# shz9/viprs

Hardware: AMD Instinct MI355X
Metric: SNP-updates/sec/E-step (1M SNPs, ~1700 LD blocks) (higher is better)
Workload: dtype f32

## Files before the change

include/viprs_hip.h:

```cpp
#ifndef VIPRS_HIP_H
#define VIPRS_HIP_H

#include <stdint.h>

#ifdef __cplusplus
extern "C" {
#endif

enum viprs_float_dtype { VIPRS_F32 = 0, VIPRS_F64 = 1 };
enum viprs_ld_dtype {
    VIPRS_LD_I8 = 0, VIPRS_LD_I16 = 1, VIPRS_LD_I32 = 2, VIPRS_LD_I64 = 3,
    VIPRS_LD_F32 = 4, VIPRS_LD_F64 = 5
};
enum viprs_indptr_dtype { VIPRS_IP_I32 = 0, VIPRS_IP_I64 = 1 };

enum viprs_status {
    VIPRS_OK = 0,
    VIPRS_EINVAL = -1,
    VIPRS_ELAYOUT = -2,
    VIPRS_EDEVICE = -3,
    VIPRS_ENOMEM = -4,
    VIPRS_EUNSUPPORTED = -5
};

// ... 104 lines not shown
int viprs_state_reset_column(viprs_state* state, int g, double pi);

int viprs_state_set_groups(viprs_state* state, int n_groups, const int64_t* group_start);
int viprs_state_prep_groups(viprs_state* state, int n, const double* params);
int viprs_state_sums_groups_begin(viprs_state* state, int n, const double* rows);
int viprs_state_sums_groups_end(viprs_state* state, double* out);
int viprs_state_prep_mixture_groups(viprs_state* state, int n, const double* params);
int viprs_state_sums_mixture_groups_begin(viprs_state* state, int n, const double* rows);
int viprs_state_sums_mixture_groups_end(viprs_state* state, double* out);
int viprs_state_prep_grid_groups(viprs_state* state, int n, const double* params);
int viprs_state_sums_grid_groups_begin(viprs_state* state, int n, const double* rows);
int viprs_state_sums_grid_groups_end(viprs_state* state, double* out);
int viprs_state_set_group_columns(viprs_state* state, int n_groups, int width, const uint8_t* active);

int viprs_state_commit_groups(viprs_state* dst, const viprs_state* src, int n, const int32_t* pairs);

#define VIPRS_COMM_ID_BYTES 128
typedef struct viprs_comm viprs_comm;
int viprs_comm_unique_id(void* id);
int viprs_comm_create(viprs_comm** comm, const void* id, int rank, int world_size, int device);
int viprs_comm_destroy(viprs_comm* comm);
int viprs_comm_rank(const viprs_comm* comm, int* rank, int* world_size);
int viprs_comm_allreduce(viprs_comm* comm, double* vec, int n, int group);
int viprs_comm_allgather(viprs_comm* comm, const double* send, int64_t n, double* recv);
int viprs_comm_barrier(viprs_comm* comm);
int viprs_state_set_comm(viprs_state* state, viprs_comm* comm);
int viprs_device_synchronize(int device);

int viprs_plan_last_kernel_ms(viprs_plan* plan, int which, double* ms);
int viprs_plan_timing_reset(viprs_plan* plan);
int viprs_plan_timing_history(viprs_plan* plan, int which, double* ms, int capacity, int* n);
int viprs_plan_last_math_modes(const viprs_plan* plan, int* mask);
int viprs_plan_last_skipped(viprs_plan* plan, int64_t* n_skipped);

int viprs_plan_dot(viprs_plan* plan, int float_dtype, int n_cols, const void* b_host, void* y_host,
                   double dq_scale, int include_diagonal);
int viprs_state_dot(viprs_state* state, int field, double dq_scale, int include_diagonal, void* y_host);
int viprs_plan_last_dot_ms(viprs_plan* plan, double* ms);

int viprs_plan_create_synthetic(viprs_plan** plan, int64_t n_blocks, const int64_t* sizes, const float* pw,
                                const float* uf0, const float* uf1, const float* sa, const float* sf, int ld_dtype,
                                int low_memory, int device);
int viprs_synthetic_ld_host(int64_t n_blocks, const int64_t* sizes, const float* pw, const float* uf0, const float* uf1,
                            const float* sa, const float* sf, int ld_dtype, int low_memory, void* out, int64_t capacity);

#ifdef __cplusplus
}
#endif
#endif
```

viprs_amd/_lib.py:

```python
import ctypes
import os

_HERE = os.path.dirname(os.path.abspath(__file__))
LIB_PATH = os.environ.get("VIPRS_HIP_LIB") or os.path.join(_HERE, "lib", "libviprs_hip.so")

F32, F64 = 0, 1
LD_I8, LD_I16, LD_I32, LD_I64, LD_F32, LD_F64 = range(6)
IP_I32, IP_I64 = 0, 1
MATH_EXACT, MATH_FAST = 0, 1
BLOCK_DENSE_SYM, BLOCK_DENSE_UPPER, BLOCK_RAGGED = 0, 1, 2
MODEL_SPIKE_SLAB, MODEL_MIXTURE, MODEL_GRID = 0, 1, 2
(FIELD_STD_BETA, FIELD_U_LOGS, FIELD_SQRT_HALF_VAR_TAU, FIELD_MU_MULT, FIELD_LOG_NULL_PI,
 FIELD_VAR_GAMMA, FIELD_VAR_MU, FIELD_ETA, FIELD_Q, FIELD_ETA_DIFF) = range(10)
(INFO_M, INFO_NNZ, INFO_N_BLOCKS, INFO_N_DENSE, INFO_N_RAGGED, INFO_MAX_BLOCK, INFO_LD_BYTES_DEVICE,
 INFO_LD_ELEM_SIZE, INFO_DEVICE, INFO_LOW_MEMORY, INFO_N_CU, INFO_UPPER_MIRRORED) = range(12)

OK, EINVAL, ELAYOUT, EDEVICE, ENOMEM, EUNSUPPORTED = 0, -1, -2, -3, -4, -5
N_SUMS = 11
COMM_ID_BYTES = 128


class ViprsHipError(RuntimeError):
    """A libviprs_hip call failed (device error, unsupported configuration...)."""

# ... 54 lines not shown
    "viprs_state_set_log_var_tau": (_i, [_vp, _vp]),
    "viprs_state_prep_mixture": (_i, [_vp, _vp, _vp, _vp, _d, _d, _d]),
    "viprs_state_sums_mixture_begin": (_i, [_vp, _d]),
    "viprs_state_sums_mixture_end": (_i, [_vp, _vp]),
    "viprs_state_prep_columns": (_i, [_vp, _i, _vp]),
    "viprs_state_sums_columns_begin": (_i, [_vp, _i, _vp]),
    "viprs_state_sums_columns_end": (_i, [_vp, _vp]),
    "viprs_state_reset_column": (_i, [_vp, _i, _d]),
    "viprs_state_set_groups": (_i, [_vp, _i, _vp]),
    "viprs_state_prep_groups": (_i, [_vp, _i, _vp]),
    "viprs_state_sums_groups_begin": (_i, [_vp, _i, _vp]),
    "viprs_state_sums_groups_end": (_i, [_vp, _vp]),
    "viprs_state_prep_mixture_groups": (_i, [_vp, _i, _vp]),
    "viprs_state_sums_mixture_groups_begin": (_i, [_vp, _i, _vp]),
    "viprs_state_sums_mixture_groups_end": (_i, [_vp, _vp]),
    "viprs_state_prep_grid_groups": (_i, [_vp, _i, _vp]),
    "viprs_state_sums_grid_groups_begin": (_i, [_vp, _i, _vp]),
    "viprs_state_sums_grid_groups_end": (_i, [_vp, _vp]),
    "viprs_state_set_group_columns": (_i, [_vp, _i, _i, _vp]),
    "viprs_state_commit_groups": (_i, [_vp, _vp, _i, _vp]),
    "viprs_comm_unique_id": (_i, [_vp]),
    "viprs_comm_create": (_i, [ctypes.POINTER(_vp), _vp, _i, _i, _i]),
    "viprs_comm_destroy": (_i, [_vp]),
    "viprs_comm_rank": (_i, [_vp, ctypes.POINTER(_i), ctypes.POINTER(_i)]),
    "viprs_comm_allreduce": (_i, [_vp, _vp, _i, _i]),
    "viprs_comm_allgather": (_i, [_vp, _vp, _i64, _vp]),
    "viprs_comm_barrier": (_i, [_vp]),
    "viprs_state_set_comm": (_i, [_vp, _vp]),
    "viprs_device_synchronize": (_i, [_i]),
    "viprs_plan_create_synthetic": (_i, [ctypes.POINTER(_vp), _i64, _vp, _vp, _vp, _vp, _vp, _vp, _i, _i, _i]),
    "viprs_synthetic_ld_host": (_i, [_i64, _vp, _vp, _vp, _vp, _vp, _vp, _i, _i, _vp, _i64]),
    "viprs_plan_last_kernel_ms": (_i, [_vp, _i, ctypes.POINTER(_d)]),
    "viprs_plan_last_skipped": (_i, [_vp, _pi64]),
    "viprs_plan_last_math_modes": (_i, [_vp, ctypes.POINTER(_i)]),
    "viprs_plan_timing_reset": (_i, [_vp]),
    "viprs_plan_timing_history": (_i, [_vp, _i, ctypes.POINTER(_d), _i, ctypes.POINTER(_i)]),
    "viprs_plan_dot": (_i, [_vp, _i, _i, _vp, _vp, _d, _i]),
    "viprs_state_dot": (_i, [_vp, _i, _d, _i, _vp]),
    "viprs_plan_last_dot_ms": (_i, [_vp, ctypes.POINTER(_d)]),
}

EXPORTED_SYMBOLS = tuple(_PROTOS)

for _name, (_res, _args) in _PROTOS.items():
    _fn = getattr(lib, _name)
    _fn.restype = _res
    _fn.argtypes = _args


def last_error():
    msg = lib.viprs_last_error()
    return msg.decode("utf-8", "replace") if msg else ""


def check(rc):
    if rc == OK:
        return
    msg = last_error()
    if rc == ELAYOUT:
        raise ViprsLayoutError(msg)
    if rc == EINVAL:
        raise ValueError(msg)
    if rc == ENOMEM:
        raise MemoryError(msg)
    if rc == EUNSUPPORTED:
        raise NotImplementedError(msg)
    raise ViprsHipError(msg)


def build_flags():
    return (lib.viprs_build_flags() or b"").decode()


def device_count():
    n = _i(0)
    rc = lib.viprs_device_count(ctypes.byref(n))
    return n.value if rc == OK else 0
```

viprs_amd/csrc/abi_estep.hip:

```cpp
#include "internal.h"

using namespace viprs;

namespace {

__global__ void sweep_prologue_kernel(int32_t* counters, int n_counters, unsigned long long* skipped,
                                      unsigned long long* granules, int64_t n_granules) {
    const int64_t i = (int64_t)blockIdx.x * blockDim.x + threadIdx.x;
    if (i < n_counters) counters[i] = 0;
    if (i == 0) { skipped[0] = 0ull; skipped[1] = 0ull; }
    for (int64_t k = i; k < n_granules; k += (int64_t)gridDim.x * blockDim.x) granules[k] = 0ull;
}

hipError_t clear_stale_skip_count(viprs_plan* P) {
    if (!P->skip_count_in_place) return hipSuccess;
    P->skip_count_in_place = false;
    return hipMemsetAsync(P->d_skipped.p, 0, sizeof(unsigned long long), P->stream);
}

template <typename T>
EStepArgs<T> make_args(viprs_state* S, double dq) {
    viprs_plan* P = S->plan;
    EStepArgs<T> A{};
    A.skipped = P->d_skipped.p;
// ... 62 lines not shown

bool use_band(const viprs_plan* P) {
    const char* f = getenv("VIPRS_BAND");
    if ((f && !atoi(f)) || P->ragged_h.empty()) return false;
    if (P->ld_dtype != VIPRS_LD_F32 && P->ld_dtype != VIPRS_LD_I8 && P->ld_dtype != VIPRS_LD_I16) return false;
    return band_ring_panels(P) <= kBandMaxRingPanels;
}

int launch_band_u(viprs_plan* P, const EStepArgs<float>& A, int model) {
    switch (P->ld_dtype) {
        case VIPRS_LD_F32: return launch_band<float>(P, A, model);
        case VIPRS_LD_I8: return launch_band<int8_t>(P, A, model);
        case VIPRS_LD_I16: return launch_band<int16_t>(P, A, model);
        default: return fail(VIPRS_EINVAL, "band schedule with unsupported LD dtype");
    }
}

int run_spike_slab(viprs_state* S, double dq) {
    viprs_plan* P = S->plan;
    HIP_TRY(hipSetDevice(P->device));
    const bool dense_only = S->float_dtype == VIPRS_F32 && !P->dense_h.empty() && P->ragged_h.empty();
    if (!dense_only) {
        const int64_t ng = P->n_granule_rows * kPanel;
        const unsigned grid = (unsigned)std::max<int64_t>(1, std::min<int64_t>((ng + 255) / 256, 1024));
        sweep_prologue_kernel<<<grid, 256, 0, P->stream>>>(P->d_counters.p, kPlanCounters, P->d_skipped.p, P->d_granules.p, ng);
        HIP_TRY(hipGetLastError());
        P->skip_count_in_place = true;
    } else {
        HIP_TRY(clear_stale_skip_count(P));
    }
    P->math_used = 0;
    hipEvent_t* ev = P->ev.data() + 4 * (P->sweeps % viprs_plan::kRing);
    P->ev_dense_only[P->sweeps % viprs_plan::kRing] = dense_only;
    if (!dense_only) HIP_TRY(hipEventRecord(ev[0], P->stream));
    int rc = VIPRS_OK;
    if (S->float_dtype == VIPRS_F32) {
        EStepArgs<float> A = make_args<float>(S, dq);
        if (!P->dense_h.empty()) {
            P->pending_start_event = ev[2];
            switch (P->ld_dtype) {
                case VIPRS_LD_F32: rc = launch_panel<float>(P, A, kPanelSpikeSlab); break;
                case VIPRS_LD_I8: rc = launch_panel<int8_t>(P, A, kPanelSpikeSlab); break;
                case VIPRS_LD_I16: rc = launch_panel<int16_t>(P, A, kPanelSpikeSlab); break;
                default: rc = fail(VIPRS_EINVAL, "dense schedule with unsupported LD dtype"); break;
            }
            if (rc != VIPRS_OK) { P->pending_start_event = nullptr; return rc; }
            HIP_TRY(hipEventRecord(ev[3], P->stream));
            P->host_t1[P->sweeps % viprs_plan::kRing] = host_clock_ms();
        }
        if (use_band(P)) rc = launch_band_u(P, A, kBandSpikeSlab);
        else if (!P->ragged_h.empty()) rc = launch_generic_u<float>(P, A, kGenSpikeSlab, false);
    } else {
        EStepArgs<double> A = make_args<double>(S, dq);
        if (!P->dense_h.empty()) { P->host_t0[P->sweeps % viprs_plan::kRing] = host_clock_ms(); HIP_TRY(hipEventRecord(ev[2], P->stream)); }
        rc = launch_tile_f64_u(P, A, kGenSpikeSlab, true);
        if (rc == VIPRS_OK && !P->dense_h.empty()) { HIP_TRY(hipEventRecord(ev[3], P->stream)); P->host_t1[P->sweeps % viprs_plan::kRing] = host_clock_ms(); }
        if (rc == VIPRS_OK) rc = launch_tile_f64_u(P, A, kGenSpikeSlab, false);
    }
    if (rc != VIPRS_OK) return rc;
    if (!dense_only) HIP_TRY(hipEventRecord(ev[1], P->stream));
    P->sweeps++;
    return VIPRS_OK;
}

static int sweep_prologue(viprs_plan* P, int n_models = 1) {
    P->skip_count_in_place = true;
// ... 5 lines not shown
    const unsigned grid = (unsigned)std::max<int64_t>(1, std::min<int64_t>((ng + 255) / 256, 1024));
    sweep_prologue_kernel<<<grid, 256, 0, P->stream>>>(P->d_counters.p, kPlanCounters, P->d_skipped.p, P->d_granules.p, ng);
    HIP_TRY(hipGetLastError());
    return VIPRS_OK;
}

static bool use_grid_mfma(const viprs_plan* P, int width) {
    if ((int64_t)P->m * std::max(1, width) >= (1LL << 31)) return false;
    if (P->grid_mfma >= 0) return P->grid_mfma != 0;
    return (int64_t)P->dense_h.size() * 8 >= (int64_t)P->n_cu * 3;
}

static int launch_grid_mfma_u(viprs_plan* P, const EStepArgs<float>& A) {
    switch (P->ld_dtype) {
        case VIPRS_LD_F32: return launch_grid_mfma<float>(P, A);
        case VIPRS_LD_I8: return launch_grid_mfma<int8_t>(P, A);
        case VIPRS_LD_I16: return launch_grid_mfma<int16_t>(P, A);
        default: return fail(VIPRS_EINVAL, "dense schedule with unsupported LD dtype");
    }
}

int run_generic_model(viprs_state* S, double dq, int model, const int32_t* d_active, int n_active,
                      const int32_t* h_active) {
    viprs_plan* P = S->plan;
    HIP_TRY(hipSetDevice(P->device));
    const bool panel_only = S->float_dtype == VIPRS_F32 && !P->dense_h.empty() && P->ragged_h.empty() &&
                            ((model == kGenMixture && S->width <= kPanelWideMaxK) || (model == kGenGrid && !use_grid_mfma(P, S->width)));
    int rc = panel_only ? VIPRS_OK : sweep_prologue(P, model == kGenGrid ? n_active : 1);
    if (rc != VIPRS_OK) return rc;
    if (panel_only) HIP_TRY(clear_stale_skip_count(P));
    P->math_used = 0;
    hipEvent_t* ev = P->ev.data() + 4 * (P->sweeps % viprs_plan::kRing);
    P->ev_dense_only[P->sweeps % viprs_plan::kRing] = true;
    {
        const bool panel_ok0 = S->float_dtype == VIPRS_F32 && !P->dense_h.empty() && (model == kGenGrid || S->width <= kPanelWideMaxK);
        if (panel_ok0) P->pending_start_event = ev[2];
        else { P->host_t0[P->sweeps % viprs_plan::kRing] = host_clock_ms(); HIP_TRY(hipEventRecord(ev[2], P->stream)); }
    }
    if (S->float_dtype == VIPRS_F32) {
        EStepArgs<float> A = make_args<float>(S, dq);
        A.active = d_active;
        A.n_active = n_active;
        if (model == kGenGrid && !S->group_cols_h.empty()) {
            A.blk_group = S->d_blk_group.p;
            A.group_cols = S->d_group_cols.p;
        }
        const int64_t lists_per_chunk = (int64_t)S->n_groups * kGroupListStride;
        const bool panel_ok = !P->dense_h.empty() && (model == kGenGrid || S->width <= kPanelWideMaxK);
        if (panel_ok && model == kGenMixture) {
            rc = launch_panel_u(P, A, S->width <= kPanelMaxK ? kPanelMixture : kPanelMixtureWide);
        } else if (panel_ok && model == kGenGrid && use_grid_mfma(P, A.width)) {
            for (int off = 0; off < n_active && rc == VIPRS_OK; off += kGridModels) {
                EStepArgs<float> Ac = A;
                Ac.active = d_active + off;
                Ac.n_active = std::min(kGridModels, n_active - off);
                if (A.group_cols) Ac.group_lists = S->d_group_lists.p + (off / kGridModels) * lists_per_chunk;
                if (off > 0) rc = sweep_prologue(P, 1);
                if (rc == VIPRS_OK) rc = launch_grid_mfma_u(P, Ac);
            }
        } else if (panel_ok && model == kGenGrid) {
            A.granules = P->d_granules.p;
            rc = launch_panel_u(P, A, kPanelGridColumn);
        } else {
            rc = launch_generic_u<float>(P, A, model, true);
        }
        if (rc == VIPRS_OK) {
// ... 270 lines not shown
```

viprs_amd/csrc/abi_plan.hip:

```cpp
#include "internal.h"
#include <chrono>

using namespace viprs;

namespace {
thread_local std::string g_err;
viprs::BuildFlagsRegistrar tu_build_flags_(VIPRS_TU_BUILD_FLAGS);
}

namespace viprs {
int fail(int code, const std::string& msg) {
    g_err = msg;
    return code;
}
SchedConfig& sched_config() {
    static SchedConfig c;
    return c;
}
static std::string& build_flags_registry() {
    static std::string s;
    return s;
}
void register_build_flags(const char* flags) {
    std::string& all = build_flags_registry();
// ... 362 lines not shown
    auto last = g_gate_plan.find(P->device);
    if (it != g_gate_event.end() && (last == g_gate_plan.end() || last->second != P))
        HIP_TRY(hipStreamWaitEvent(P->stream, it->second, 0));
    return VIPRS_OK;
}
void team_launch_forget(const viprs_plan* P) {
    std::lock_guard<std::mutex> lock(g_gate_mutex);
    auto last = g_gate_plan.find(P->device);
    if (last != g_gate_plan.end() && last->second == P) g_gate_plan.erase(last);
}
int team_launch_done(viprs_plan* P) {
    std::lock_guard<std::mutex> lock(g_gate_mutex);
    auto it = g_gate_event.find(P->device);
    if (it == g_gate_event.end()) {
        hipEvent_t e = nullptr;
        HIP_TRY(hipEventCreateWithFlags(&e, hipEventDisableTiming));
        it = g_gate_event.emplace(P->device, e).first;
    }
    HIP_TRY(hipEventRecord(it->second, P->stream));
    g_gate_plan[P->device] = P;
    return VIPRS_OK;
}
int plan_create_generated(viprs_plan** out, int64_t m, const int32_t* lb, const std::vector<int64_t>& ip64, int ld_dtype,
                          int low_memory, int device, const std::function<int(void*)>& fill) {
    return plan_create_impl(out, m, lb, ip64, nullptr, ld_dtype, low_memory, device, nullptr, &fill);
}
}

extern "C" {

const char* viprs_last_error(void) { return g_err.c_str(); }
const char* viprs_version(void) { return "viprs_amd 0.1.0 (gfx950)"; }
const char* viprs_build_flags(void) { return build_flags_registry().c_str(); }

int viprs_device_count(int* count) {
    if (!count) return fail(VIPRS_EINVAL, "count is null");
    int n = 0;
    hipError_t e = hipGetDeviceCount(&n);
    if (e != hipSuccess) { *count = 0; return fail(VIPRS_EDEVICE, hipGetErrorString(e)); }
    *count = n;
    return VIPRS_OK;
}

int viprs_host_fingerprint(const void* data, int64_t n_bytes, uint64_t* out) {
    if (!out || n_bytes < 0 || (n_bytes > 0 && !data)) return fail(VIPRS_EINVAL, "bad argument");
    const unsigned char* b = static_cast<const unsigned char*>(data);
    uint64_t h = 0x9e3779b97f4a7c15ull ^ (uint64_t)n_bytes;
    auto mix = [&](const unsigned char* p, int64_t n) {
        int64_t i = 0;
        for (; i + 8 <= n; i += 8) {
            uint64_t w;
            std::memcpy(&w, p + i, 8);
            h = (h ^ w) * 0xff51afd7ed558ccdull;
            h ^= h >> 32;
        }
        for (; i < n; ++i) { h = (h ^ p[i]) * 0x100000001b3ull; }
    };
    constexpr int64_t kEdge = 4096, kSamples = 256, kWin = 64;
    if (n_bytes <= 2 * kEdge + kSamples * kWin) {
        mix(b, n_bytes);
    } else {
        mix(b, kEdge);
        mix(b + n_bytes - kEdge, kEdge);
        const int64_t step = (n_bytes - kWin) / kSamples;
        for (int64_t k = 0; k < kSamples; ++k) mix(b + k * step, kWin);
    }
// ... 181 lines not shown
```

viprs_amd/csrc/estep_panel.h:

```cpp
#pragma once
#include <type_traits>

#include "device_math.h"
#include "kernels_common.h"

#ifndef PANEL_MIN_WAVES
#define PANEL_MIN_WAVES 2
#endif

namespace viprs {

#ifdef VIPRS_SWEEP_TRACE
__device__ unsigned long long g_sweep_trace[1 << 15][4];
__device__ unsigned int g_sweep_trace_n;
#endif

#ifdef VIPRS_PANEL_PROFILE
#define PPROF(slot, cond) do { if (TEAM && item == 0 && member < 2 && lane == 0 && p < 64 && (cond)) s_pprof[p][slot] = (unsigned)wall_clock64(); } while (0)
#else
#define PPROF(slot, cond) do { } while (0)
#endif

template <typename U> __device__ __forceinline__ float4 load4(const U* p);
template <> __device__ __forceinline__ float4 load4<float>(const float* p) {
// ... 131 lines not shown
template <typename U, int CPL, bool FULL, int DEPTH = kStripRowsInFlight, bool MIXED = false>
__device__ __forceinline__ void strip_update(const U* __restrict__ rowp, int stride, int last_row, float avec,
                                             float* __restrict__ lq_c, float fvec = 1.0f) {
    static_assert(kPanel % DEPTH == 0, "panel must be a whole number of prefetch groups");
    float qv[CPL];
#pragma unroll
    for (int i = 0; i < CPL; ++i) qv[i] = lq_c[i];
    RawRow<U, CPL> buf[DEPTH];
#pragma unroll
    for (int k = 0; k < DEPTH; ++k)
        buf[k] = load_raw<U, CPL>(rowp + (int64_t)(FULL ? k : min(k, last_row)) * stride);
#pragma unroll 1
    for (int g = 0; g < kPanel / DEPTH - 1; ++g) {
#pragma unroll
        for (int k = 0; k < DEPTH; ++k) {
            const RawRow<U, CPL> v = buf[k];
            const int rn = DEPTH * (g + 1) + k;
            buf[k] = load_raw<U, CPL>(rowp + (int64_t)(FULL ? rn : min(rn, last_row)) * stride);
            const float a = MIXED ? fvec * rl(avec, DEPTH * g + k) : rl(avec, DEPTH * g + k);
#pragma unroll
            for (int i = 0; i < CPL; ++i) qv[i] = __builtin_fmaf(v.get(i), a, qv[i]);
            __builtin_amdgcn_sched_barrier(0);
        }
    }
#pragma unroll
    for (int k = 0; k < DEPTH; ++k) {
        const RawRow<U, CPL> v = buf[k];
        const float a = MIXED ? fvec * rl(avec, kPanel - DEPTH + k) : rl(avec, kPanel - DEPTH + k);
#pragma unroll
        for (int i = 0; i < CPL; ++i) qv[i] = __builtin_fmaf(v.get(i), a, qv[i]);
    }
#pragma unroll
    for (int i = 0; i < CPL; ++i) lq_c[i] = qv[i];
}

__device__ __forceinline__ float diag_lower_update(const float* __restrict__ tile, float edvec, float sv, int lane) {
#pragma unroll 16
    for (int jr = 0; jr < kPanel; ++jr) {
        const float t = __builtin_fmaf(tile[jr * kPanel + lane], rl(edvec, jr), sv);
        sv = lane < jr ? t : sv;
    }
    return sv;
}

template <bool EXACT>
struct SpikeSlabModel {
    static constexpr bool kLaneParallel = false;
    struct In { float mm, beta, sv, ulog, eta_old; };
    static __device__ __forceinline__ In load(const EStepArgs<float>& A, int64_t j, bool live) {
        In in;
        in.mm = live ? A.mu_mult[j] : 0.0f;
        in.beta = live ? A.std_beta[j] : 0.0f;
        in.sv = live ? A.shvt[j] : 0.0f;
        in.ulog = live ? A.u_logs[j] : 0.0f;
        in.eta_old = live ? A.eta[j] : 0.0f;
        return in;
    }
    static constexpr bool kHasSkip = true;
    template <int LOOKUP>
    static __device__ __forceinline__ float delta(const In& in, float q, const ExpTab& tab, int sel) {
        float mu, gamma, d;
        snp_update<EXACT, LOOKUP>(in.mm, in.beta, in.sv, in.ulog, in.eta_old, q, tab, mu, gamma, d, sel);
        return d;
    }
    template <int LOOKUP>
    static __device__ __forceinline__ bool update(const In& in, float q, const ExpTab& tab, float& d, int sel) {
// ... 45 lines not shown
        gamma = EXACT ? sigmoid_exact<LOOKUP>(u, tab, sel) : sigmoid_fast(u);
        d = gamma * mu - in.eta_old;
    }
    static constexpr bool kHasSkip = false;
    template <int LOOKUP>
    static __device__ __forceinline__ float delta(const In& in, float q, const ExpTab& tab, int sel) {
        float mu, gamma, d;
        core<LOOKUP>(in, q, tab, mu, gamma, d, sel);
        return d;
    }
    template <int LOOKUP>
    static __device__ __forceinline__ bool update(const In& in, float q, const ExpTab& tab, float& d, int sel) {
        d = delta<LOOKUP>(in, q, tab, sel);
        return true;
    }
    template <bool TEAM>
    static __device__ __forceinline__ float finish(const EStepArgs<float>& A, int64_t j, const In& in, float q,
                                                   const ExpTab& tab, bool live, bool writer, bool& skipped,
                                                   float* d_out = nullptr) {
        float mu, gamma, d;
        core<kLookupPerLane>(in, q, tab, mu, gamma, d, 0);
        if (d_out) *d_out = live ? d : 0.0f;
        if (live && writer) {
            A.var_mu[j] = mu;
            A.var_gamma[j] = gamma;
            A.eta_diff[j] = d;
            if (TEAM) stage_store(A.eta_out + j, in.eta_old + d); else A.eta[j] = in.eta_old + d;
        }
        skipped = false;
        return live ? A.dq * d : 0.0f;
    }
};

template <typename MODEL> struct IsGridColumn : std::false_type {};
template <bool EXACT> struct IsGridColumn<GridColumnModel<EXACT>> : std::true_type {};

template <bool EXACT, int LOOKUP>
__device__ __forceinline__ float softmax_exp(float x, const ExpTab& tab, int sel = 0) {
    if constexpr (EXACT) return expf_glibc_nonpos<LOOKUP>(x, tab, sel);
    else return expf_fast_nonpos(x);
}
template <bool EXACT>
__device__ __forceinline__ float softmax_div(float e, float ssum) {
    if constexpr (EXACT) return e / ssum;
    else return e * __builtin_amdgcn_rcpf(ssum);
}

template <bool EXACT = true>
struct MixtureModel {
    static constexpr bool kExact = EXACT;
    static constexpr bool kLaneParallel = true;
    struct In { float mm[kPanelMaxK], sv[kPanelMaxK], ulog[kPanelMaxK]; float lnp, beta, eta_old; int K; };
    static __device__ __forceinline__ In load(const EStepArgs<float>& A, int64_t j, bool live) {
        In in;
        in.K = A.width;
#pragma unroll
        for (int k = 0; k < kPanelMaxK; ++k) {
            const bool on = live && k < in.K;
            const int64_t idx = on ? j * in.K + k : 0;
            in.mm[k] = on ? A.mu_mult[idx] : 0.0f;
            in.sv[k] = on ? A.shvt[idx] : 0.0f;
            in.ulog[k] = on ? A.u_logs[idx] : 0.0f;
        }
        in.lnp = live ? A.log_null_pi[j] : 0.0f;
        in.beta = live ? A.std_beta[j] : 0.0f;
        in.eta_old = live ? A.eta[j] : 0.0f;
// ... 66 lines not shown
    static __device__ __forceinline__ In load(const EStepArgs<float>& A, int64_t j, bool live) {
        In in;
        in.K = A.width;
        in.lnp = live ? A.log_null_pi[j] : 0.0f;
        in.beta = live ? A.std_beta[j] : 0.0f;
        in.eta_old = live ? A.eta[j] : 0.0f;
        return in;
    }
};
template <typename M, typename = void> struct is_wide_mixture { static constexpr bool value = false; };
template <typename M> struct is_wide_mixture<M, std::enable_if_t<M::kWide>> { static constexpr bool value = true; };

constexpr int kFormSym = 1, kFormMirror = 2;

template <typename U, typename MODEL, int FORM, int NW, bool TEAM, int CPL>
__device__ __forceinline__ void panel_role(const EStepArgs<float>& A0, const int qcap, float* __restrict__ smem, const int wg) {
    constexpr bool MIR = FORM == kFormMirror;
    constexpr bool SUMS = FORM != kFormSym;
    constexpr bool kDiagInLds = !MODEL::kLaneParallel;
    constexpr bool kMixLds = MODEL::kLaneParallel;
    constexpr bool kStageDiag = kDiagInLds || kMixLds;
    float* lq = smem;
    float* la = smem + qcap;
    float* lT = la + 2 * kPanel;
    float* lTo = lT + 2 * kPanel * kPanel;
    float* lmx = lTo + kPanel * kPanel;
    float* led = lmx + ((MODEL::kLaneParallel && !is_wide_mixture<MODEL>::value) ? kMixLdsFloats : 0);
    float* ls = led + 2 * kPanel;
#ifdef PANEL_TEAM_STRIP_DEPTH
    constexpr int kDepth = TEAM ? PANEL_TEAM_STRIP_DEPTH : kStripRowsInFlight;
#else
    constexpr int kDepth = TEAM ? (kPanel / RawRow<U, CPL>::kWords < kPanel ? kPanel / RawRow<U, CPL>::kWords : kPanel) : kStripRowsInFlight;
#endif
    __shared__ int s_blk;
    __shared__ int s_tdone;
    __shared__ int s_ddone;

    const int tid = threadIdx.x;
    const int wave = __builtin_amdgcn_readfirstlane(tid >> 6);
    const int lane = tid & 63;
    const U* __restrict__ ldd = static_cast<const U*>(A0.ld_dense);
    ExpTab tab;
    tab.init();
    unsigned long long my_skipped = 0;
    const float dq = A0.dq;
    const int n_models = max(1, A0.n_active);

    constexpr int kSW = kPanel * CPL;
    const int TS = TEAM ? A0.team_size : 1;
    const int team = TEAM ? wg / TS : 0;
    const int member = TEAM ? wg % TS : 0;
    int team_iter = 0;

    for (;;) {
        int item;
        if (TEAM) {
            item = team + team_iter * A0.n_teams;
            ++team_iter;
        } else {
            if (tid == 0) {
                int it = atomicAdd(A0.counter, 1);
                if (A0.bottom_mod > 0 && it < A0.n_blocks * n_models) {
                    const bool bottom = (wg % A0.bottom_mod) == A0.bottom_mod - 1;
                    it = bottom ? A0.n_blocks * n_models - 1 - atomicAdd(A0.counter + 2, 1) : atomicAdd(A0.counter + 1, 1);
                }
                s_blk = it;
// ... 430 lines not shown
                        v[g] = load4<U>(base + (int64_t)min(row_base + row, b - 1) * stride + (p + 1) * kPanel + tcol);
                    }
                    float4 w[kGroups];
                    {
#pragma unroll
                        for (int g = 0; g < kGroups; ++g) {
                            const int row = 4 * min(uw + g * (NW - 1), kPanel / 4 - 1) + trow;
                            w[g] = load4<U>(base + (int64_t)min(p * kPanel + row, b - 1) * stride + (p + 1) * kPanel + tcol);
                        }
                    }
                    if (MIR && p > 0) {
                        while (*reinterpret_cast<volatile int*>(&s_ddone) < p) __builtin_amdgcn_s_sleep(1);
                    }
#pragma unroll
                    for (int g = 0; g < kGroups; ++g) {
                        const int i = uw + g * (NW - 1);
                        if (i < kPanel / 4) *reinterpret_cast<float4*>(T + (4 * i + trow) * kPanel + tcol) = v[g];
                    }
                    {
                        while (*reinterpret_cast<volatile int*>(&s_tdone) < p + 1) __builtin_amdgcn_s_sleep(1);
#pragma unroll
                        for (int g = 0; g < kGroups; ++g) {
                            const int i = uw + g * (NW - 1);
                            if (i < kPanel / 4) *reinterpret_cast<float4*>(lTo + (4 * i + trow) * kPanel + tcol) = w[g];
                        }
                    }
                }
                };
                const int pp = p - 1;
                const int rr0 = pp * kPanel;
                const int last_row = min(kPanel, b - rr0) - 1;
                const float avec = p > 0 ? la[(pp & 1) * kPanel + lane] : 0.0f;
                const int nstrips = (bpad + kSW - 1) / kSW;
                const bool any_a = __ballot(avec != 0.0f) != 0;
                const float edvec = (MIR && p > 0) ? led[(pp & 1) * kPanel + lane] : 0.0f;
                const bool any_ed = MIR && __ballot(edvec != 0.0f) != 0;
                const int s_pri = ((p + 1) * kPanel) / kSW;
                const int n_mine = (nstrips - member + TS - 1) / TS;
                auto do_strip = [&](int k) {
                    int st = member + k * TS, kl = k;
                    if (TEAM) {
                        const int k_pri = (s_pri % TS == member) ? (s_pri - member) / TS : 0;
                        kl = (k + k_pri) % n_mine;
                        st = member + kl * TS;
                    }
                    const int c = st * kSW + CPL * lane;
                    float* __restrict__ lq_c = lq + (TEAM ? kl * kSW + CPL * lane : c);
                    const int cp = c >> 6;
#if defined(PANEL_TIMING_NO_SECOND_PASS) && PANEL_TIMING_NO_SECOND_PASS + 0 >= 2
                    const bool active = (c < b) && cp > p;
#else
                    const bool active = (c < b) && cp != pp && cp != p;
#endif
                    auto hand_off = [&]() {
                        if (TEAM && st == s_pri && p + 1 < np && p + 1 >= 2) {
                            __builtin_amdgcn_wave_barrier();
                            const float v = lq[loc((p + 1) * kPanel + lane)];
                            const unsigned long long g =
                                ((unsigned long long)(A.tag_base + (unsigned)(p + 2)) << 32) | (unsigned long long)__float_as_uint(v);
                            __hip_atomic_store(gran + (int64_t)(p + 1) * kPanel + lane, g, __ATOMIC_RELAXED,
                                               __HIP_MEMORY_SCOPE_AGENT);
                        }
                    };
                    if constexpr (MIR) {
                        const bool left = cp < pp;
                        float* __restrict__ tgt = left ? ls + (TEAM ? kl * kSW + CPL * lane : c) : lq_c;
                        const bool any_l = __ballot(active && left) != 0, any_r = __ballot(active && !left) != 0;
                        if (any_l && any_r) {
                            const float fvec = left ? 1.0f : dq;
                            if (any_ed && active) {
                                if (last_row == kPanel - 1)
                                    strip_update<U, CPL, true, kDepth, true>(base + (int64_t)rr0 * stride + c, stride, last_row, edvec, tgt, fvec);
                                else
                                    strip_update<U, CPL, false, kDepth, true>(base + (int64_t)rr0 * stride + c, stride, last_row, edvec, tgt, fvec);
                            }
                        } else {
                            float mvec = any_l ? edvec : avec;
                            asm volatile("" : "+v"(mvec));
                            if ((any_l ? any_ed : any_a) && active) {
                                if (last_row == kPanel - 1)
                                    strip_update<U, CPL, true, kDepth>(base + (int64_t)rr0 * stride + c, stride, last_row, mvec, tgt);
                                else
                                    strip_update<U, CPL, false, kDepth>(base + (int64_t)rr0 * stride + c, stride, last_row, mvec, tgt);
                            }
                        }
                        if (k == uw) PPROF(6, wave == 1);
                        hand_off();
                    } else {
                        if (any_a && active) {
                            if (last_row == kPanel - 1)
                                strip_update<U, CPL, true, kDepth>(base + (int64_t)rr0 * stride + c, stride, last_row, avec, lq_c);
                            else
                                strip_update<U, CPL, false, kDepth>(base + (int64_t)rr0 * stride + c, stride, last_row, avec, lq_c);
                        }
                        if (k == uw) PPROF(6, wave == 1);
                        hand_off();
                    }
                };
                if (MIR && p > 0 && uw == NW - 2) {
#ifdef PANEL_TIMING_NO_SECOND_PASS
                    if (false) {
#else
                    if (any_ed && own(rr0)) {
#endif
                        float* __restrict__ sp = ls + loc(rr0 + lane);
                        *sp = diag_lower_update(lT + (pp & 1) * kPanel * kPanel, edvec, *sp, lane);
                    }
                    if (lane == 0) *reinterpret_cast<volatile int*>(&s_ddone) = p;
                }
                stage_tiles();
                PPROF(5, wave == 1);
                if (p > 0) {
                    for (int k = uw; k < n_mine; k += NW - 1) do_strip(k);
                }
            }
            PPROF(7, wave == 1);
            __syncthreads();
        }
        }
#ifdef VIPRS_PANEL_PROFILE
        if (TEAM && item == 0 && member < 2 && tid == 0) {
            for (int p = 0; p < np && p < 64; p += (p < 4 || p > np - 4) ? 1 : 8) {
                const unsigned t = s_pprof[p][0];
// ... 83 lines not shown
```

viprs_amd/csrc/kernels_common.h:

```cpp
#pragma once
#include <hip/hip_runtime.h>
#include <stdint.h>

#if (defined(PANEL_TIMING_NO_HANDOFF_WAIT) || \
    defined(PANEL_TIMING_NO_SECOND_PASS) || \
    defined(PANEL_NW) || \
    defined(PANEL_STRIP_DEPTH) || \
    defined(PANEL_MIN_WAVES) || \
    defined(PANEL_TEAM_STRIP_DEPTH) || \
    defined(PANEL_TEAM_CPL_F32) || \
    defined(PANEL_CHAIN_PRIO) || \
    defined(VIPRS_GRID_MFMA_CHAIN) || \
    defined(VIPRS_GRID_PROFILE) || \
    defined(VIPRS_TILE_PROFILE) || \
    defined(VIPRS_SWEEP_TRACE) || \
    defined(VIPRS_PANEL_PROFILE)) && \
    !defined(VIPRS_EXPERIMENTAL)
#error "experiment switch defined without -DVIPRS_EXPERIMENTAL (see kernels_common.h)"
#endif
#ifdef VIPRS_EXPERIMENTAL
#define VIPRS_BF_VIPRS_EXPERIMENTAL " VIPRS_EXPERIMENTAL"
#else
#define VIPRS_BF_VIPRS_EXPERIMENTAL ""
#endif
#ifdef PANEL_TIMING_NO_HANDOFF_WAIT
#define VIPRS_BF_PANEL_TIMING_NO_HANDOFF_WAIT " PANEL_TIMING_NO_HANDOFF_WAIT"
#else
#define VIPRS_BF_PANEL_TIMING_NO_HANDOFF_WAIT ""
#endif
#ifdef PANEL_TIMING_NO_SECOND_PASS
#define VIPRS_BF_PANEL_TIMING_NO_SECOND_PASS " PANEL_TIMING_NO_SECOND_PASS"
#else
#define VIPRS_BF_PANEL_TIMING_NO_SECOND_PASS ""
#endif
#ifdef PANEL_NW
#define VIPRS_BF_PANEL_NW " PANEL_NW"
#else
#define VIPRS_BF_PANEL_NW ""
#endif
#ifdef PANEL_STRIP_DEPTH
#define VIPRS_BF_PANEL_STRIP_DEPTH " PANEL_STRIP_DEPTH"
#else
#define VIPRS_BF_PANEL_STRIP_DEPTH ""
#endif
#ifdef PANEL_MIN_WAVES
#define VIPRS_BF_PANEL_MIN_WAVES " PANEL_MIN_WAVES"
#else
#define VIPRS_BF_PANEL_MIN_WAVES ""
#endif
#ifdef PANEL_TEAM_STRIP_DEPTH
#define VIPRS_BF_PANEL_TEAM_STRIP_DEPTH " PANEL_TEAM_STRIP_DEPTH"
#else
#define VIPRS_BF_PANEL_TEAM_STRIP_DEPTH ""
#endif
#ifdef PANEL_TEAM_CPL_F32
#define VIPRS_BF_PANEL_TEAM_CPL_F32 " PANEL_TEAM_CPL_F32"
#else
#define VIPRS_BF_PANEL_TEAM_CPL_F32 ""
#endif
#ifdef PANEL_CHAIN_PRIO
#define VIPRS_BF_PANEL_CHAIN_PRIO " PANEL_CHAIN_PRIO"
#else
#define VIPRS_BF_PANEL_CHAIN_PRIO ""
#endif
#ifdef VIPRS_GRID_MFMA_CHAIN
#define VIPRS_BF_VIPRS_GRID_MFMA_CHAIN " VIPRS_GRID_MFMA_CHAIN"
#else
#define VIPRS_BF_VIPRS_GRID_MFMA_CHAIN ""
#endif
#ifdef VIPRS_GRID_PROFILE
#define VIPRS_BF_VIPRS_GRID_PROFILE " VIPRS_GRID_PROFILE"
#else
#define VIPRS_BF_VIPRS_GRID_PROFILE ""
#endif
#ifdef VIPRS_TILE_PROFILE
#define VIPRS_BF_VIPRS_TILE_PROFILE " VIPRS_TILE_PROFILE"
#else
#define VIPRS_BF_VIPRS_TILE_PROFILE ""
#endif
#ifdef VIPRS_SWEEP_TRACE
#define VIPRS_BF_VIPRS_SWEEP_TRACE " VIPRS_SWEEP_TRACE"
#else
#define VIPRS_BF_VIPRS_SWEEP_TRACE ""
#endif
#ifdef VIPRS_PANEL_PROFILE
#define VIPRS_BF_VIPRS_PANEL_PROFILE " VIPRS_PANEL_PROFILE"
#else
#define VIPRS_BF_VIPRS_PANEL_PROFILE ""
#endif
#define VIPRS_TU_BUILD_FLAGS VIPRS_BF_VIPRS_EXPERIMENTAL VIPRS_BF_PANEL_TIMING_NO_HANDOFF_WAIT VIPRS_BF_PANEL_TIMING_NO_SECOND_PASS VIPRS_BF_PANEL_NW VIPRS_BF_PANEL_STRIP_DEPTH VIPRS_BF_PANEL_MIN_WAVES VIPRS_BF_PANEL_TEAM_STRIP_DEPTH VIPRS_BF_PANEL_TEAM_CPL_F32 VIPRS_BF_PANEL_CHAIN_PRIO VIPRS_BF_VIPRS_GRID_MFMA_CHAIN VIPRS_BF_VIPRS_GRID_PROFILE VIPRS_BF_VIPRS_TILE_PROFILE VIPRS_BF_VIPRS_SWEEP_TRACE VIPRS_BF_VIPRS_PANEL_PROFILE

namespace viprs {
void register_build_flags(const char* flags);
struct BuildFlagsRegistrar { explicit BuildFlagsRegistrar(const char* f) { register_build_flags(f); } };
}

namespace viprs {

constexpr int kPanel = 64;
constexpr int kStrip = 256;

__host__ __device__ constexpr int panel_lds_floats(int qcap, bool offdiag_tile = false) {
    return qcap + 2 * kPanel + 2 * kPanel * kPanel + (offdiag_tile ? kPanel * kPanel : 0);
}
__host__ __device__ constexpr int panel_mirror_lds_floats(int qcap) { return 2 * kPanel + qcap; }
constexpr int kPanelMaxK = 8;
constexpr int kPanelWideMaxK = 31;
constexpr int kMixLdsFloats = 5 * kPanel * kPanelMaxK;
constexpr int kMaxMixtureK = 64;
constexpr int kGridModels = 32;
constexpr int kGridResOwners = 6, kGridResSlots = 2;
constexpr int kGridResMaxCols = kGridResOwners * kGridResSlots * 2 * kPanel;
constexpr int kBandMaxRingPanels = 256;

struct BlockDesc {
    int32_t start;
    int32_t size;
    int32_t stride;
    int32_t kind;
    int64_t ld_off;
    int64_t gr_off;
    int32_t band_left;
    int32_t band_right;
};

template <typename T>
struct EStepArgs {
    const BlockDesc* blocks;
    int32_t n_blocks;
    int32_t* counter;
    int32_t bottom_mod;
    unsigned long long* granules;
    uint32_t tag_base;
// ... 50 lines not shown
```

Baseline: 1.569 billion.

## Skip zero-multiplier rows in panel strip updates via compact ballot row walk

For the spike-slab model, the panel kernel now takes a ballot of which panel rows have nonzero update multipliers. When few enough rows are live, it walks only those rows in prefetched groups instead of streaming all 64 LD rows. This targets the LD-row memory traffic and FMAs spent on rows whose coefficient is zero. The cost is bit-scan overhead, extra registers for the group buffers, and a new build knob for group size.

```diff
diff --git a/include/viprs_hip.h b/include/viprs_hip.h
--- a/include/viprs_hip.h
+++ b/include/viprs_hip.h
@@ -160,6 +160,7 @@
 int viprs_plan_timing_history(viprs_plan* plan, int which, double* ms, int capacity, int* n);
 int viprs_plan_last_math_modes(const viprs_plan* plan, int* mask);
 int viprs_plan_last_skipped(viprs_plan* plan, int64_t* n_skipped);
+int viprs_panel_skip_group(void);
 
 int viprs_plan_dot(viprs_plan* plan, int float_dtype, int n_cols, const void* b_host, void* y_host,
                    double dq_scale, int include_diagonal);
diff --git a/viprs_amd/_lib.py b/viprs_amd/_lib.py
--- a/viprs_amd/_lib.py
+++ b/viprs_amd/_lib.py
@@ -110,6 +110,7 @@
     "viprs_synthetic_ld_host": (_i, [_i64, _vp, _vp, _vp, _vp, _vp, _vp, _i, _i, _vp, _i64]),
     "viprs_plan_last_kernel_ms": (_i, [_vp, _i, ctypes.POINTER(_d)]),
     "viprs_plan_last_skipped": (_i, [_vp, _pi64]),
+    "viprs_panel_skip_group": (_i, []),
     "viprs_plan_last_math_modes": (_i, [_vp, ctypes.POINTER(_i)]),
     "viprs_plan_timing_reset": (_i, [_vp]),
     "viprs_plan_timing_history": (_i, [_vp, _i, ctypes.POINTER(_d), _i, ctypes.POINTER(_i)]),
@@ -120,7 +121,11 @@
 
 EXPORTED_SYMBOLS = tuple(_PROTOS)
 
+_OPTIONAL = ("viprs_panel_skip_group",)
+
 for _name, (_res, _args) in _PROTOS.items():
+    if _name in _OPTIONAL and not hasattr(lib, _name):
+        continue
     _fn = getattr(lib, _name)
     _fn.restype = _res
     _fn.argtypes = _args
@@ -150,6 +155,10 @@
     return (lib.viprs_build_flags() or b"").decode()
 
 
+def panel_skip_group():
+    return int(lib.viprs_panel_skip_group()) if hasattr(lib, "viprs_panel_skip_group") else 0
+
+
 def device_count():
     n = _i(0)
     rc = lib.viprs_device_count(ctypes.byref(n))
diff --git a/viprs_amd/csrc/abi_estep.hip b/viprs_amd/csrc/abi_estep.hip
--- a/viprs_amd/csrc/abi_estep.hip
+++ b/viprs_amd/csrc/abi_estep.hip
@@ -118,6 +118,7 @@
     P->math_used = 0;
     hipEvent_t* ev = P->ev.data() + 4 * (P->sweeps % viprs_plan::kRing);
     P->ev_dense_only[P->sweeps % viprs_plan::kRing] = dense_only;
+    P->host_t0[P->sweeps % viprs_plan::kRing] = P->host_t1[P->sweeps % viprs_plan::kRing] = 0.0;
     if (!dense_only) HIP_TRY(hipEventRecord(ev[0], P->stream));
     int rc = VIPRS_OK;
     if (S->float_dtype == VIPRS_F32) {
@@ -189,6 +190,7 @@
     P->math_used = 0;
     hipEvent_t* ev = P->ev.data() + 4 * (P->sweeps % viprs_plan::kRing);
     P->ev_dense_only[P->sweeps % viprs_plan::kRing] = true;
+    P->host_t0[P->sweeps % viprs_plan::kRing] = P->host_t1[P->sweeps % viprs_plan::kRing] = 0.0;
     {
         const bool panel_ok0 = S->float_dtype == VIPRS_F32 && !P->dense_h.empty() && (model == kGenGrid || S->width <= kPanelWideMaxK);
         if (panel_ok0) P->pending_start_event = ev[2];
diff --git a/viprs_amd/csrc/abi_plan.hip b/viprs_amd/csrc/abi_plan.hip
--- a/viprs_amd/csrc/abi_plan.hip
+++ b/viprs_amd/csrc/abi_plan.hip
@@ -418,6 +418,7 @@
 const char* viprs_last_error(void) { return g_err.c_str(); }
 const char* viprs_version(void) { return "viprs_amd 0.1.0 (gfx950)"; }
 const char* viprs_build_flags(void) { return build_flags_registry().c_str(); }
+int viprs_panel_skip_group(void) { return viprs::kSkipGroup; }
 
 int viprs_device_count(int* count) {
     if (!count) return fail(VIPRS_EINVAL, "count is null");
diff --git a/viprs_amd/csrc/estep_panel.h b/viprs_amd/csrc/estep_panel.h
--- a/viprs_amd/csrc/estep_panel.h
+++ b/viprs_amd/csrc/estep_panel.h
@@ -187,6 +187,69 @@
     }
 #pragma unroll
     for (int i = 0; i < CPL; ++i) lq_c[i] = qv[i];
+}
+
+template <typename U, int CPL, int G, bool MIXED = false>
+__device__ __forceinline__ void strip_update_compact(const U* __restrict__ rowu, unsigned coff, int stride, unsigned long long rows,
+                                                     float avec, float* __restrict__ lq_c, float fvec = 1.0f) {
+    float qv[CPL];
+#pragma unroll
+    for (int i = 0; i < CPL; ++i) qv[i] = lq_c[i];
+    const int r_pad = 63 - __builtin_clzll(rows);
+    const int ngroups = (__popcll(rows) + G - 1) / G;
+    unsigned long long ml = rows, mc = rows;
+    auto next_row = [&](unsigned long long& m) {
+        const int r = m ? __builtin_ctzll(m) : r_pad;
+        m &= m - 1;
+        return r;
+    };
+    auto next_mult = [&]() {
+        const bool on = mc != 0;
+        const float a = rl(avec, next_row(mc));
+        return MIXED ? fvec * (on ? a : 0.0f) : (on ? a : 0.0f);
+    };
+    RawRow<U, CPL> buf[G];
+#pragma unroll
+    for (int k = 0; k < G; ++k) buf[k] = load_raw<U, CPL>(rowu + (int64_t)next_row(ml) * stride + coff);
+#pragma unroll 1
+    for (int g = 1; g < ngroups; ++g) {
+#pragma unroll
+        for (int k = 0; k < G; ++k) {
+            const RawRow<U, CPL> v = buf[k];
+            buf[k] = load_raw<U, CPL>(rowu + (int64_t)next_row(ml) * stride + coff);
+            const float a = next_mult();
+#pragma unroll
+            for (int i = 0; i < CPL; ++i) qv[i] = __builtin_fmaf(v.get(i), a, qv[i]);
+            __builtin_amdgcn_sched_barrier(0);
+        }
+    }
+#pragma unroll
+    for (int k = 0; k < G; ++k) {
+        const RawRow<U, CPL> v = buf[k];
+        const float a = next_mult();
+#pragma unroll
+        for (int i = 0; i < CPL; ++i) qv[i] = __builtin_fmaf(v.get(i), a, qv[i]);
+    }
+#pragma unroll
+    for (int i = 0; i < CPL; ++i) lq_c[i] = qv[i];
+}
+
+template <int DEPTH> __host__ __device__ constexpr int skip_group() {
+    return kSkipGroup * DEPTH / 16 > 0 ? kSkipGroup * DEPTH / 16 : 1;
+}
+
+template <typename U, int CPL, int DEPTH, bool MIXED = false>
+__device__ __forceinline__ void strip_apply(const U* __restrict__ rowu, int c, int stride, int last_row, unsigned long long rows,
+                                            float mvec, float* __restrict__ tgt, float fvec = 1.0f) {
+    constexpr int G = skip_group<DEPTH>();
+    const int n = __popcll(rows);
+    if (G < kPanel && (n + G - 1) / G * G < kPanel) {
+        strip_update_compact<U, CPL, G, MIXED>(rowu, (unsigned)c, stride, rows, mvec, tgt, fvec);
+    } else if (last_row == kPanel - 1) {
+        strip_update<U, CPL, true, DEPTH, MIXED>(rowu + c, stride, last_row, mvec, tgt, fvec);
+    } else {
+        strip_update<U, CPL, false, DEPTH, MIXED>(rowu + c, stride, last_row, mvec, tgt, fvec);
+    }
 }
 
 __device__ __forceinline__ float diag_lower_update(const float* __restrict__ tile, float edvec, float sv, int lane) {
@@ -298,6 +361,8 @@
     }
 };
 
+template <typename MODEL> struct HasSkipBranch : std::false_type {};
+template <bool EXACT> struct HasSkipBranch<SpikeSlabModel<EXACT>> : std::true_type {};
 template <typename MODEL> struct IsGridColumn : std::false_type {};
 template <bool EXACT> struct IsGridColumn<GridColumnModel<EXACT>> : std::true_type {};
 
@@ -430,6 +495,7 @@
 #else
     constexpr int kDepth = TEAM ? (kPanel / RawRow<U, CPL>::kWords < kPanel ? kPanel / RawRow<U, CPL>::kWords : kPanel) : kStripRowsInFlight;
 #endif
+    constexpr bool kSkipRows = HasSkipBranch<MODEL>::value;
     __shared__ int s_blk;
     __shared__ int s_tdone;
     __shared__ int s_ddone;
@@ -926,9 +992,12 @@
                 const int last_row = min(kPanel, b - rr0) - 1;
                 const float avec = p > 0 ? la[(pp & 1) * kPanel + lane] : 0.0f;
                 const int nstrips = (bpad + kSW - 1) / kSW;
-                const bool any_a = __ballot(avec != 0.0f) != 0;
+                const unsigned long long live_rows = ~0ull >> (kPanel - 1 - last_row);
+                const unsigned long long rows_a = kSkipRows ? __ballot(avec != 0.0f) & live_rows : 0ull;
+                const bool any_a = kSkipRows ? rows_a != 0 : __ballot(avec != 0.0f) != 0;
                 const float edvec = (MIR && p > 0) ? led[(pp & 1) * kPanel + lane] : 0.0f;
-                const bool any_ed = MIR && __ballot(edvec != 0.0f) != 0;
+                const unsigned long long rows_ed = (MIR && kSkipRows) ? __ballot(edvec != 0.0f) & live_rows : 0ull;
+                const bool any_ed = kSkipRows ? rows_ed != 0 : MIR && __ballot(edvec != 0.0f) != 0;
                 const int s_pri = ((p + 1) * kPanel) / kSW;
                 const int n_mine = (nstrips - member + TS - 1) / TS;
                 auto do_strip = [&](int k) {
@@ -963,7 +1032,9 @@
                         if (any_l && any_r) {
                             const float fvec = left ? 1.0f : dq;
                             if (any_ed && active) {
-                                if (last_row == kPanel - 1)
+                                if constexpr (kSkipRows)
+                                    strip_apply<U, CPL, kDepth, true>(base + (int64_t)rr0 * stride, c, stride, last_row, rows_ed, edvec, tgt, fvec);
+                                else if (last_row == kPanel - 1)
                                     strip_update<U, CPL, true, kDepth, true>(base + (int64_t)rr0 * stride + c, stride, last_row, edvec, tgt, fvec);
                                 else
                                     strip_update<U, CPL, false, kDepth, true>(base + (int64_t)rr0 * stride + c, stride, last_row, edvec, tgt, fvec);
@@ -972,7 +1043,9 @@
                             float mvec = any_l ? edvec : avec;
                             asm volatile("" : "+v"(mvec));
                             if ((any_l ? any_ed : any_a) && active) {
-                                if (last_row == kPanel - 1)
+                                if constexpr (kSkipRows)
+                                    strip_apply<U, CPL, kDepth>(base + (int64_t)rr0 * stride, c, stride, last_row, any_l ? rows_ed : rows_a, mvec, tgt);
+                                else if (last_row == kPanel - 1)
                                     strip_update<U, CPL, true, kDepth>(base + (int64_t)rr0 * stride + c, stride, last_row, mvec, tgt);
                                 else
                                     strip_update<U, CPL, false, kDepth>(base + (int64_t)rr0 * stride + c, stride, last_row, mvec, tgt);
@@ -982,7 +1055,9 @@
                         hand_off();
                     } else {
                         if (any_a && active) {
-                            if (last_row == kPanel - 1)
+                            if constexpr (kSkipRows)
+                                strip_apply<U, CPL, kDepth>(base + (int64_t)rr0 * stride, c, stride, last_row, rows_a, avec, lq_c);
+                            else if (last_row == kPanel - 1)
                                 strip_update<U, CPL, true, kDepth>(base + (int64_t)rr0 * stride + c, stride, last_row, avec, lq_c);
                             else
                                 strip_update<U, CPL, false, kDepth>(base + (int64_t)rr0 * stride + c, stride, last_row, avec, lq_c);
diff --git a/viprs_amd/csrc/kernels_common.h b/viprs_amd/csrc/kernels_common.h
--- a/viprs_amd/csrc/kernels_common.h
+++ b/viprs_amd/csrc/kernels_common.h
@@ -8,6 +8,7 @@
     defined(PANEL_STRIP_DEPTH) || \
     defined(PANEL_MIN_WAVES) || \
     defined(PANEL_TEAM_STRIP_DEPTH) || \
+    defined(PANEL_SKIP_GROUP) || \
     defined(PANEL_TEAM_CPL_F32) || \
     defined(PANEL_CHAIN_PRIO) || \
     defined(VIPRS_GRID_MFMA_CHAIN) || \
@@ -53,6 +54,12 @@
 #else
 #define VIPRS_BF_PANEL_TEAM_STRIP_DEPTH ""
 #endif
+#ifdef PANEL_SKIP_GROUP
+#define VIPRS_BF_PANEL_SKIP_GROUP " PANEL_SKIP_GROUP"
+#else
+#define VIPRS_BF_PANEL_SKIP_GROUP ""
+#define PANEL_SKIP_GROUP 8
+#endif
 #ifdef PANEL_TEAM_CPL_F32
 #define VIPRS_BF_PANEL_TEAM_CPL_F32 " PANEL_TEAM_CPL_F32"
 #else
@@ -88,7 +95,7 @@
 #else
 #define VIPRS_BF_VIPRS_PANEL_PROFILE ""
 #endif
-#define VIPRS_TU_BUILD_FLAGS VIPRS_BF_VIPRS_EXPERIMENTAL VIPRS_BF_PANEL_TIMING_NO_HANDOFF_WAIT VIPRS_BF_PANEL_TIMING_NO_SECOND_PASS VIPRS_BF_PANEL_NW VIPRS_BF_PANEL_STRIP_DEPTH VIPRS_BF_PANEL_MIN_WAVES VIPRS_BF_PANEL_TEAM_STRIP_DEPTH VIPRS_BF_PANEL_TEAM_CPL_F32 VIPRS_BF_PANEL_CHAIN_PRIO VIPRS_BF_VIPRS_GRID_MFMA_CHAIN VIPRS_BF_VIPRS_GRID_PROFILE VIPRS_BF_VIPRS_TILE_PROFILE VIPRS_BF_VIPRS_SWEEP_TRACE VIPRS_BF_VIPRS_PANEL_PROFILE
+#define VIPRS_TU_BUILD_FLAGS VIPRS_BF_VIPRS_EXPERIMENTAL VIPRS_BF_PANEL_TIMING_NO_HANDOFF_WAIT VIPRS_BF_PANEL_TIMING_NO_SECOND_PASS VIPRS_BF_PANEL_NW VIPRS_BF_PANEL_STRIP_DEPTH VIPRS_BF_PANEL_MIN_WAVES VIPRS_BF_PANEL_TEAM_STRIP_DEPTH VIPRS_BF_PANEL_SKIP_GROUP VIPRS_BF_PANEL_TEAM_CPL_F32 VIPRS_BF_PANEL_CHAIN_PRIO VIPRS_BF_VIPRS_GRID_MFMA_CHAIN VIPRS_BF_VIPRS_GRID_PROFILE VIPRS_BF_VIPRS_TILE_PROFILE VIPRS_BF_VIPRS_SWEEP_TRACE VIPRS_BF_VIPRS_PANEL_PROFILE
 
 namespace viprs {
 void register_build_flags(const char* flags);
@@ -99,6 +106,8 @@
 
 constexpr int kPanel = 64;
 constexpr int kStrip = 256;
+constexpr int kSkipGroup = PANEL_SKIP_GROUP;
+static_assert(kSkipGroup == 4 || kSkipGroup == 8 || kSkipGroup == 16, "rows per group of the compact row walk");
 
 __host__ __device__ constexpr int panel_lds_floats(int qcap, bool offdiag_tile = false) {
     return qcap + 2 * kPanel + 2 * kPanel * kPanel + (offdiag_tile ? kPanel * kPanel : 0);
```

New measurement: 1.551 billion. -1.2%, worse.
